# lzhLab/kmcEx

Hardware: AMD Instinct MI355X
Metric: k-mers/s encoded (insert) + k-mers/s queried, k=31 nh=7; % HBM-BW roofline (higher is better)
Workload: dtype u64; 1 GPU; synthetic 100000000 distinct canonical 31-mers per GPU, D1 counts, insert then query (110000000 queries: all inserted k-mers shuffled, half reverse-complemented, +10% absent); k=31, nh=7, nb=5, ci=1, cs=1023, kmers_per_gpu=100000000

## Files before the change

kmcex_amd/csrc/kernels.hip:

```cpp
#include "launchers.h"
#include <cstdlib>

__constant__ u32 c_seeds[128] = {
	46757, 46769, 46771, 46807, 46811, 46817, 46819, 46829, 46831, 46853, 46861, 46867, 46877, 46889, 46901, 46919,
	46933, 46957, 46993, 46997, 47017, 47041, 47051, 47057, 47059, 47087, 47093, 47111, 47119, 47123, 47129, 47137,
	47143, 47147, 47149, 47161, 47189, 47207, 47221, 47237, 47251, 47269, 47279, 47287, 47293, 47297, 47303, 47309,
	47317, 47339, 47351, 47353, 47363, 47381, 47387, 47389, 47407, 47417, 47419, 47431, 47441, 47459, 47491, 47497,
	47501, 47507, 47513, 47521, 47527, 47533, 47543, 47563, 47569, 47581, 47591, 47599, 47609, 47623, 47629, 47639,
	47653, 47657, 47659, 47681, 47699, 47701, 47711, 47713, 47717, 47737, 47741, 47743, 47777, 47779, 47791, 47797,
	47807, 47809, 47819, 47837, 47843, 47857, 47869, 47881, 47903, 47911, 47917, 47933, 47939, 47947, 47951, 47963,
	47969, 47977, 47981, 48017, 48023, 48029, 48049, 48073, 48079, 48091, 48109, 48119, 48121, 48131, 48157, 48163};

template <int W> __device__ __forceinline__ void load_kmer(const u64 *base, u64 i, u64 *v)
{
#pragma unroll
	for (int w = 0; w < W; w++) v[w] = base[i * W + w];
}
template <int W> __device__ __forceinline__ void store_kmer(u64 *base, u64 i, const u64 *v)
{
#pragma unroll
	for (int w = 0; w < W; w++) base[i * W + w] = v[w];
}

template <int W> __device__ __forceinline__ void bloom_insert_pm(const Premixed<W> &pm, const StrGeom g, u32 *bits, const ModU64 md, int nhash)
// ... 1198 lines not shown
		for (int r = 0; r < RPT; r++) {
			if (!mine[r] && !ghost[r]) continue;
			const u32 pub = mine[r] ? resv[r] : (ghost[r] & hold[r]);
			u32 later = mine[r] ? 0u : (ghost[r] & ~hold[r]);
#pragma unroll
			for (int j = 0; j < NHM; j++)
				if (j < md.nh && ((pub >> j) & 1u)) {
					const u64 q = FIN_Q(r, j);
					u32 *slot = ((second[r] >> j) & 1u) ? s_t2 + fin_slot2(q) : s_t1 + fin_slot1(q);
					const u32 cur = *slot, mark = FIN_MARK | fin_ident(q) | (((bin[r] >> j) & 1u) << 30);
					if (!(cur & FIN_MARK)) *slot = mark;
					else if ((cur & 0x3FFFFFu) == fin_ident(q)) *slot = cur | mark;
					else later |= 1u << j;
				}
			if (mine[r]) {
				if (!defer) {
#pragma unroll
					for (int j = 0; j < NHM; j++)
						if (j < md.nh && ((resv[r] >> j) & 1u)) {
							const u32 b = FIN_BIT(r, j);
							atomicOr(cells + cidx[r][j], CELL_TAG(b) | (((bin[r] >> j) & 1u) ? CELL_VAL(b) : 0u));
						}
				}
				bd.status[pp][row + x[r]] = SLOT_INSERTED;
				live[r] = false;
				won[r] = true;
				succ++;
			}
			ghost[r] = later;
			if (later) s_pending[par] = 1;
			__builtin_amdgcn_sched_barrier(0);
		}
		lds_barrier();
#pragma unroll
		for (int r = 0; r < RPT; r++) {
			if (!live[r]) continue;
			bool conflict = false;
#pragma unroll
			for (int j = 0; j < NHM; j++)
				if (j < md.nh && ((resv[r] >> j) & 1u)) {
					const u64 q = FIN_Q(r, j);
					const u32 m = ((second[r] >> j) & 1u) ? s_t2[fin_slot2(q)] : s_t1[fin_slot1(q)];
					if ((m & FIN_MARK) && (m & 0x3FFFFFu) == fin_ident(q)) {
						conflict |= ((m >> 30) & 1u) != ((bin[r] >> j) & 1u);
						um[r] &= ~(1u << j);
					}
				}
			if (conflict) { mark_failed(bd, pp, i, row, x[r]); live[r] = false; }
			else s_pending[par] = 1;
			__builtin_amdgcn_sched_barrier(0);
		}
		lds_barrier();
#pragma unroll
		for (int r = 0; r < RPT; r++)
#pragma unroll
			for (int j = 0; j < NHM; j++)
				if (j < md.nh && ((resv[r] >> j) & 1u)) {
					const u64 q = FIN_Q(r, j);
					s_t1[fin_slot1(q)] = 0;
					if ((second[r] >> j) & 1u) s_t2[fin_slot2(q)] = 0;
				}
		lds_barrier();
		if (!s_pending[par]) break;
	}
#undef FIN_BIT
#undef FIN_Q
#pragma unroll
	for (int r = 0; r < RPT; r++)
		if (won[r] && defer) bd.Urec[lv][(row + rec[r]) * (1 + W)] |= REC_WON;
	if (!defer) drain_vmem();
	if (succ) atomicAdd(s_succ, succ);
	return iters + 1;
}

template <int W, int NHM, int RPT>
__device__ __forceinline__ void finish_lds_ranges(const ModelDev &md, const BlockDev &bd, int pp, int i, int a, int lv, int n, bool snapshot,
                                                   u32 *s_t1, u32 *s_t2, u32 *s_list, int *s_count, int *s_pending, int *s_succ)
{
	constexpr int CAP = RPT * 1024;
	const u64 row = (u64)i * KMX_BUCKET;
	for (int q = threadIdx.x; q < KMX_FIN_T; q += 1024) { s_t1[q] = 0; s_t2[q] = 0; }
	u64 iters = 0;
	if (n <= CAP) {
		__syncthreads();
		iters = finish_lds<W, NHM, RPT>(md, bd, pp, i, a, lv, n, nullptr, snapshot, true, s_t1, s_t2, s_pending, s_succ);
	} else {
		const int n_list = bd.n[pp][i];
		int lo = 0, remaining = n;
		while (remaining > 0) {
			int hi = n_list;
			if (remaining > CAP) hi = lo + max(1, (int)((long long)(n_list - lo) * (CAP * 7 / 8) / remaining));
			int cnt;
			for (;;) {
				if (threadIdx.x == 0) *s_count = 0;
				__syncthreads();
				for (int u = threadIdx.x; u < n; u += 1024) {
					const int x = (int)((u32)bd.Urec[lv][(row + u) * (1 + W)] & (KMX_BUCKET - 1));
					if (x >= lo && x < hi) {
						const int slot = atomicAdd(s_count, 1);
						if (slot < CAP) s_list[slot] = (u32)u;
					}
				}
				__syncthreads();
				cnt = *s_count;
				__syncthreads();
				if (cnt <= CAP) break;
				hi = lo + max(1, (hi - lo) / 2);
			}
			iters += finish_lds<W, NHM, RPT>(md, bd, pp, i, a, lv, cnt, s_list, snapshot && lo == 0, false, s_t1, s_t2, s_pending, s_succ);
			__syncthreads();
			if (threadIdx.x == 0) s_pending[0] = 0;
			remaining -= cnt;
			lo = hi;
			if (lo >= n_list) break;
		}
	}
	__syncthreads();
	if (threadIdx.x == 0) {
		atomicAdd(bd.stats + ST_FIN_ITERS, iters);
		if (*s_succ) atomicAdd(bd.stats + ST_SLOW_SUCC, (u64)*s_succ);
	}
}

template <int W, int NHM>
__device__ __forceinline__ void finish_global(const ModelDev &md, const BlockDev &bd, int pp, int i, int a, int lv, int n, bool first, u64 epoch_b, u64 epoch0,
                                               int *s_pending, int *s_succ)
{
	const u64 row = (u64)i * KMX_BUCKET;
	u64 epoch = epoch0;
	u64 iters = 0;
	for (;; iters++) {
		if (threadIdx.x == 0) *s_pending = 0;
		__syncthreads();
		if (!first) {
			for (int u = threadIdx.x; u < n; u += 1024) {
				u32 x, bin;
				u64 v[W];
				rec_load<W>(bd.Urec[lv], row + u, x, bin, v);
				if (bd.status[pp][row + x] != SLOT_UNDECIDED) continue;
				Premixed<W> pm = premix_string<W>(left_align<W>(v, md.k), md.gfull);
				Touches<NHM> tc;
				gather_touches<W, NHM, true>(md, pm, a, tc);
				if (touches_conflict<NHM>(md, tc, bin)) { mark_failed(bd, pp, i, row, x); continue; }
				reserve_untagged<NHM>(md, bd, i, tc, resv_key(epoch, x));
				*s_pending = 1;
			}
			drain_vmem();
			__syncthreads();
			const int pending = *s_pending;
			__syncthreads();
			if (!pending) break;
		}
		int succ = 0;
		for (int u = threadIdx.x; u < n; u += 1024) {
			u32 x, bin;
			u64 v[W];
			const u32 um = rec_load<W>(bd.Urec[lv], row + u, x, bin, v);
			if (bd.status[pp][row + x] != SLOT_UNDECIDED) continue;
			Aligned<W> al = left_align<W>(v, md.k);
			Premixed<W> pm = premix_string<W>(al, md.gfull);
			if (first) {
				const u64 key = resv_key(epoch_b, x);
				const int sbase = a * md.nh;
				cell_t *cells = md.cells[a];
				u64 pos[NHM];
				bool mine = true;
#pragma unroll
				for (int j = 0; j < NHM; j++)
					if (j < md.nh && ((um >> j) & 1u)) {
						pos[j] = mod_u64(murmur_seeded<W>(pm, md.gfull, c_seeds[(sbase + j) & 127]), md.km_mod);
						mine &= cell_load_coherent(resv_slot(bd, i, pos[j])) == key;
					}
				if (mine) {
#pragma unroll
					for (int j = 0; j < NHM; j++)
						if (j < md.nh && ((um >> j) & 1u)) {
							const u32 b = bit_in_cell(pos[j]);
							atomicOr(cells + (pos[j] >> 4), CELL_TAG(b) | (value_at_position<NHM>(md, pos, um, bin, j) ? CELL_VAL(b) : 0u));
						}
					bd.status[pp][row + x] = SLOT_INSERTED;
					succ++;
				}
				continue;
			}
			Touches<NHM> tc;
			gather_touches<W, NHM, true>(md, pm, a, tc);
			if (owns_outcome<NHM, true>(md, bd, i, tc, bin, resv_key(epoch, x))) {
				commit_touches<W, NHM>(md, tc, bin, a);
				bd.status[pp][row + x] = SLOT_INSERTED;
				succ++;
			}
		}
		if (succ) atomicAdd(s_succ, succ);
		drain_vmem();
		__syncthreads();
		if (!first) epoch++;
		first = false;
	}
	if (threadIdx.x == 0) {
		atomicAdd(bd.stats + ST_FIN_ITERS, iters);
		if (*s_succ) atomicAdd(bd.stats + ST_SLOW_SUCC, (u64)*s_succ);
	}
}

template <int W, int NHM> __global__ __launch_bounds__(1024) void k_slow_finish(ModelDev md, BlockDev bd, int t, int pp, int s, u64 epoch_b, u64 epoch0, int force_global, KmbackJob job, BitScatter kmb)
{
	constexpr int RKPT = KMX_FIN_RIDER_KPT(NHM);
	constexpr int FIN_BYTES = (2 * KMX_FIN_T + KMX_FIN_RPT(NHM) * 1024) * 4 + 8 * 4, RIDER_BYTES = BS_LDS_BYTES(RKPT * (NHM - 2), 1024);
	__shared__ __align__(16) unsigned char pool[FIN_BYTES > RIDER_BYTES ? FIN_BYTES : RIDER_BYTES];
	if ((int)blockIdx.x >= md.nb) {
		const int r = (int)blockIdx.x - md.nb, gxk = KMX_BUCKET / (1024 * RKPT);
		kmback_emit_body<W, NHM, RKPT, 1024>(md, bd, job.kmers, job.surv, pp, job.n_in_block, kmb, job.i0 + r / gxk, r % gxk, gxk, pool);
		return;
	}
	u32 *s_t1 = (u32 *)pool, *s_t2 = s_t1 + KMX_FIN_T, *s_list = s_t2 + KMX_FIN_T;
	int *s_pending = (int *)(s_list + KMX_FIN_RPT(NHM) * 1024);
	int &s_succ = s_pending[3], &s_count = s_pending[4];
	const int i = blockIdx.x, lv = s & 1;
	const int n = bd.Un[UN_IDX(lv, i, md.nb)];
	if (n == 0) return;
	const int a = (i + t) % md.nb;
	constexpr int RPT = KMX_FIN_RPT(NHM);
	const bool lds_path = n <= KMX_FIN_RANGES * RPT * 1024 && !force_global && md.km_mod.d < KMX_FIN_MAX_POS;
	if (threadIdx.x == 0) {
		s_succ = 0;
		s_pending[0] = 0;
		atomicMax(bd.stats + ST_MAX_UFIN, (u64)n);
		if (s == 0) { atomicAdd(bd.stats + ST_CONTENDED, (u64)n); atomicMax(bd.stats + ST_MAX_U0, (u64)n); }
	}
	__syncthreads();
	const bool snap = s == 0 && snapshot_ok(bd, i);
	if (lds_path) finish_lds_ranges<W, NHM, RPT>(md, bd, pp, i, a, lv, n, snap, s_t1, s_t2, s_list, &s_count, s_pending, &s_succ);
	else finish_global<W, NHM>(md, bd, pp, i, a, lv, n, snap, epoch_b, epoch0, s_pending, &s_succ);
}

template <int W, int NHM> __global__ __launch_bounds__(256) void k_reorder(ModelDev md, BlockDev bd, int t, int pp, int lv)
{
	__shared__ int s_tmp[4];
	__shared__ int s_m, s_off;
	const int nb = md.nb;
	const int i = blockIdx.y, tile = blockIdx.x;
	const int n = bd.n[pp][i];
	const u64 row = (u64)i * KMX_BUCKET;
	if (tile >= (int)KMX_NTILES) {
		const int nrec = bd.Un[UN_IDX(lv, i, nb)];
		for (int u = (tile - (int)KMX_NTILES) * 256 + threadIdx.x; u < nrec; u += KMX_APPLY_WGS * 256) {
			const u64 *rec = bd.Urec[lv] + (row + u) * (1 + W);
			if (rec[0] & REC_WON) {
				const int a = (i + t) % nb;
				u32 x, bin;
				u64 v[W];
				rec_load<W>(bd.Urec[lv], row + u, x, bin, v);
				Aligned<W> al = left_align<W>(v, md.k);
				Premixed<W> pm = premix_string<W>(al, md.gfull);
				cell_t *cells = md.cells[a];
#pragma unroll
				for (int j = 0; j < NHM; j++)
					if (j < md.nh) {
						const u64 pos = mod_u64(murmur_seeded<W>(pm, md.gfull, c_seeds[(a * md.nh + j) & 127]), md.km_mod);
						const u32 b = bit_in_cell(pos);
						atomicOr(cells + (pos >> 4), CELL_TAG(b) | (((bin >> j) & 1u) ? CELL_VAL(b) : 0u));
					}
			}
		}
		return;
	}
	{
		int c = bd.tile_cnt[pp][i * KMX_NTILES + threadIdx.x];
		int tot;
		int ex = block_excl_scan_256(c, s_tmp, &tot);
		if ((int)threadIdx.x == tile) s_off = ex;
		if (threadIdx.x == 0) s_m = tot;
		__syncthreads();
	}
	const int m = s_m;
	int f[4], c = 0;
#pragma unroll
	for (int q = 0; q < 4; q++) {
		int x = tile * KMX_TILE + threadIdx.x * 4 + q;
		f[q] = (x < n && bd.status[pp][row + x] == SLOT_FAILED) ? 1 : 0;
		c += f[q];
	}
	int before = block_excl_scan_256(c, s_tmp, nullptr) + s_off;
	const u32 *oldl = bd.list[pp] + row;
	u32 *newl = bd.list[pp ^ 1] + row;
	u32 *mv = bd.mover[pp ^ 1] + row;
#pragma unroll
	for (int q = 0; q < 4; q++) {
		int x = tile * KMX_TILE + threadIdx.x * 4 + q;
		if (x < n) {
			if (x < m) newl[x] = f[q] ? oldl[x] : (LIST_HOLE | (u32)(x - before));
			else if (f[q]) mv[m - before - 1] = oldl[x];
		}
		before += f[q];
	}
	bd.tile_cnt[pp ^ 1][i * KMX_NTILES + tile] = 0;
	if (tile == 0 && threadIdx.x == 0) {
		bd.cl_ovf[i] = 0;
		if (n > m) atomicAdd(bd.stats + ST_SUCCESSES, (u64)(n - m));
		bd.n[pp ^ 1][i] = m;
	}
}

__global__ __launch_bounds__(1024) void k_bs_apply(BitScatter bs)
{
	__shared__ u32 s_tile[BS_TILE_WORDS];
	const u32 TW = 1u << (bs.tlog2 - 5);
	const u32 b = blockIdx.x;
	u32 cnt = (u32)bs.cnt[b];
	if (cnt == 0) return;
	if (cnt > bs.cap) cnt = bs.cap;
	const u64 wpb = 1ULL << (bs.wshift - 5), word0 = (u64)b * wpb;
	if (word0 >= bs.nwords) return;
	const u32 nw = (u32)((bs.nwords - word0) < wpb ? (bs.nwords - word0) : wpb);
	const u32 *tup = bs.tup + (u64)b * bs.cap;
	u32 *words = bs.words + word0;
	for (u32 t0 = 0; t0 < nw; t0 += TW) {
		const u32 tw = nw - t0 < TW ? nw - t0 : TW;
		for (u32 w = threadIdx.x; w < tw; w += 1024) s_tile[w] = 0;
		__syncthreads();
		for (u32 q = threadIdx.x; q < cnt; q += 1024) {
			const u32 o = tup[q], w = (o >> 5) - t0;
			if (w < tw) atomicOr(&s_tile[w], 1u << (o & 31));
		}
		__syncthreads();
		for (u32 w = threadIdx.x; w < tw; w += 1024) {
			const u32 x = s_tile[w];
			if (x) words[t0 + w] |= x;
		}
		__syncthreads();
	}
	if (threadIdx.x == 0) bs.cnt[b] = 0;
}

#define BS_SPLIT_K 8
__global__ __launch_bounds__(256) void k_bs_split(BitScatter bs)
{
	__shared__ int s_cnt[1 << BS_MAX_TILES_LOG2], s_off[1 << BS_MAX_TILES_LOG2], s_base[1 << BS_MAX_TILES_LOG2], s_tmp[4];
	__shared__ u32 s_stage[256 * BS_SPLIT_K];
	const u32 b = blockIdx.y, tl = bs.wshift - bs.tlog2, tmask = (1u << bs.tlog2) - 1;
	u32 cnt = (u32)bs.cnt[b];
	if (cnt > bs.cap) cnt = bs.cap;
	const u32 *tup = bs.tup + (u64)b * bs.cap;
	u32 *out = bs.tup2 + (((u64)b << tl) * bs.cap2);
	int *gcnt = bs.cnt2 + ((u64)b << tl);
	for (u32 base = blockIdx.x * (256 * BS_SPLIT_K); base < cnt; base += gridDim.x * (256 * BS_SPLIT_K)) {
		s_cnt[threadIdx.x] = 0;
		__syncthreads();
		u32 o[BS_SPLIT_K];
		int rank[BS_SPLIT_K];
#pragma unroll
		for (int j = 0; j < BS_SPLIT_K; j++) {
			const u32 q = base + j * 256 + threadIdx.x;
			o[j] = q < cnt ? tup[q] : ~0u;
		}
#pragma unroll
		for (int j = 0; j < BS_SPLIT_K; j++)
			if (o[j] != ~0u) rank[j] = atomicAdd(&s_cnt[o[j] >> bs.tlog2], 1);
		__syncthreads();
		int total;
		{
			const int c = s_cnt[threadIdx.x];
			const int ex = block_excl_scan_256(c, s_tmp, &total);
			s_off[threadIdx.x] = ex;
			s_base[threadIdx.x] = c ? atomicAdd(gcnt + threadIdx.x, c) : 0;
		}
		__syncthreads();
#pragma unroll
		for (int j = 0; j < BS_SPLIT_K; j++)
			if (o[j] != ~0u) s_stage[s_off[o[j] >> bs.tlog2] + rank[j]] = o[j];
		__syncthreads();
		for (int q = threadIdx.x; q < total; q += 256) {
			const u32 e = s_stage[q], t = e >> bs.tlog2;
			const u32 g = (u32)s_base[t] + (u32)(q - s_off[t]);
			if (g < bs.cap2) out[(u64)t * bs.cap2 + g] = e & tmask;
			else atomicOr(bs.words + (((u64)b << bs.wshift) >> 5) + (e >> 5), 1u << (e & 31));
		}
		__syncthreads();
	}
}
__global__ __launch_bounds__(1024) void k_bs_apply2(BitScatter bs)
{
	__shared__ u32 s_tile[BS_TILE_WORDS];
	const u32 b = blockIdx.y, t = blockIdx.x, tl = bs.wshift - bs.tlog2, TW = 1u << (bs.tlog2 - 5);
	int *gc = bs.cnt2 + (((u64)b << tl) + t);
	u32 cnt = (u32)*gc;
	if (t == 0 && threadIdx.x == 0) bs.cnt[b] = 0;
	if (cnt == 0) return;
	if (cnt > bs.cap2) cnt = bs.cap2;
	const u64 word0 = (((u64)b << bs.wshift) >> 5) + (u64)t * TW;
	if (word0 >= bs.nwords) { if (threadIdx.x == 0) *gc = 0; return; }
	const u32 tw = (u32)((bs.nwords - word0) < TW ? (bs.nwords - word0) : TW);
	const u32 *tup = bs.tup2 + (((u64)b << tl) + t) * bs.cap2;
	u32 *words = bs.words + word0;
	for (u32 w = threadIdx.x; w < tw; w += 1024) s_tile[w] = 0;
	__syncthreads();
	for (u32 q = threadIdx.x; q < cnt; q += 1024) {
		const u32 o = tup[q];
		if ((o >> 5) < tw) atomicOr(&s_tile[o >> 5], 1u << (o & 31));
	}
	__syncthreads();
	for (u32 w = threadIdx.x; w < tw; w += 1024) {
		const u32 x = s_tile[w];
		if (x) words[w] |= x;
	}
	if (threadIdx.x == 0) *gc = 0;
}

template <int W, int NHM, int KPT, int BT>
__device__ __forceinline__ void kmback_emit_body(const ModelDev &md, const BlockDev &bd, const u64 *kmers, const unsigned char *surv, int pp, int n_in_block,
                                                 const BitScatter &bs, int i, int bx, int gx, unsigned char *lds)
{
	constexpr int K = KPT * (NHM - 2);
	BS_LDS_AT(K, BT, lds);
	const bool whole = n_in_block >= 0;
	int n;
	if (whole) { n = n_in_block - i * (int)KMX_BUCKET; n = n < 0 ? 0 : (n > (int)KMX_BUCKET ? (int)KMX_BUCKET : n); }
	else n = bd.n[pp][i];
	const u64 row = (u64)i * KMX_BUCKET;
	for (int base = bx * BT * KPT; base < n; base += gx * BT * KPT) {
		u64 v[K];
		u32 valid = 0;
#pragma unroll
		for (int q = 0; q < KPT; q++) {
			const int x = base + q * BT + (int)threadIdx.x;
			if (x < n && (whole ? !surv[row + x] : bd.status[pp][row + x] != SLOT_FAILED)) {
				const u32 idx = whole ? (u32)x : bd.list[pp][row + x];
				u64 km[W];
				load_kmer<W>(kmers, row + idx, km);
				Premixed<W> pb = premix_string<W>(drop_first_base<W>(left_align<W>(km, md.k)), md.gback);
				if (md.kmb_direct) {
					bloom_insert_pm<W>(pb, md.gback, md.km_back, md.km_back_mod, md.nh - 2);
					continue;
				}
#pragma unroll
				for (int j = 0; j < NHM - 2; j++)
					if (j < md.nh - 2) {
						const u64 pos = mod_u64(murmur_seeded<W>(pb, md.gback, c_seeds[j]), md.km_back_mod);
						v[q * (NHM - 2) + j] = ((pos >> 5) << 5) | bit_in_word32(pos);
						valid |= 1u << (q * (NHM - 2) + j);
					}
			}
		}
		if (!md.kmb_direct) bs_block_emit<K, BT>(bs, v, valid, s_bs_cnt, s_bs_off, s_bs_base, s_bs_tmp, s_bs_stage);
	}
}
template <int W, int NHM, int KPT> __global__ __launch_bounds__(256) void k_kmback_emit(ModelDev md, BlockDev bd, const u64 *kmers, const unsigned char *surv, int i0, int istride, int pp, int n_in_block, BitScatter bs)
{
	__shared__ __align__(16) unsigned char lds[BS_LDS_BYTES(KPT * (NHM - 2), 256)];
	kmback_emit_body<W, NHM, KPT>(md, bd, kmers, surv, pp, n_in_block, bs, i0 + (int)blockIdx.y * istride, (int)blockIdx.x, (int)gridDim.x, lds);
}

template <int W> __global__ __launch_bounds__(256) void k_rest_append(BlockDev bd, int pp, int i0, int istride, u64 *rest_kmers, int *rest_counts, unsigned long long *rest_n, u64 *stale_kmers, int *stale_counts, u64 *feedback)
{
	__shared__ int s_cnt;
	__shared__ unsigned long long s_base;
	if (blockIdx.x == 0 && blockIdx.y == 0 && threadIdx.x == 0) {
		feedback[0] = bd.stats[ST_MAX_U0]; feedback[1] = bd.stats[ST_MAX_UFIN]; feedback[2] = bd.stats[ST_MAX_LATE_BIN];
		bd.stats[ST_MAX_U0] = 0; bd.stats[ST_MAX_UFIN] = 0; bd.stats[ST_MAX_LATE_BIN] = 0;
	}
	if (threadIdx.x == 0) s_cnt = 0;
	__syncthreads();
	const int i = i0 + (int)blockIdx.y * istride, x = blockIdx.x * 256 + threadIdx.x;
	const int n = bd.n[pp][i];
	if (x == 0 && n == 0) stale_counts[i] = 0;
	const bool act = x < n;
	const u64 mask = __ballot(act);
	const int lane = threadIdx.x & 63;
	int wbase = 0;
	if (lane == 0 && mask) wbase = atomicAdd(&s_cnt, (int)__popcll(mask));
	wbase = __shfl(wbase, 0, 64);
	__syncthreads();
	if (threadIdx.x == 0) s_base = s_cnt ? atomicAdd(rest_n, (unsigned long long)s_cnt) : 0ULL;
	__syncthreads();
	if (!act) return;
	const u64 p = s_base + (u64)wbase + (u64)__popcll(mask & ((1ULL << lane) - 1));
	const u64 row = (u64)i * KMX_BUCKET;
	const u32 idx = list_entry(bd, pp, row, x);
	u64 v[W];
	load_kmer<W>(bd.kmers, row + idx, v);
	const int c = (int)bd.counts[row + idx];
	store_kmer<W>(rest_kmers, p, v);
	rest_counts[p] = c;
	bd.surv[row + idx] = 1;
	if (x == 0) { store_kmer<W>(stale_kmers, (u64)i, v); stale_counts[i] = c; }
}

template <int W> __global__ __launch_bounds__(256) void k_ring_import(BlockDev bd, int nb, int pp, RingLists rl, u64 *stg_kmers, u32 *stg_counts)
{
	const int i = blockIdx.y, x = blockIdx.x * 256 + threadIdx.x;
	const RingList e = rl.e[i];
	const u64 row = (u64)i * KMX_BUCKET;
	int n = 0;
	if (e.active) {
		const u64 *src_k = e.n_host >= 0 ? e.src_kmers : e.src_msg + KMX_MSG_HDR;
		const u32 *src_c = e.n_host >= 0 ? e.src_counts : (const u32 *)(e.src_msg + KMX_MSG_HDR + (u64)KMX_BUCKET * W);
		n = e.n_host >= 0 ? e.n_host : (int)e.src_msg[0];
		n = n < 0 ? 0 : (n > (int)KMX_BUCKET ? (int)KMX_BUCKET : n);
		if (x < n) {
			u64 v[W];
			load_kmer<W>(src_k, (u64)x, v);
			store_kmer<W>(stg_kmers, row + x, v);
			stg_counts[row + x] = src_c[x];
		}
		bd.list[pp][row + x] = (u32)x;
		bd.surv[row + x] = 0;
	}
	if (x < (int)KMX_NTILES) { bd.tile_cnt[0][i * KMX_NTILES + x] = 0; bd.tile_cnt[1][i * KMX_NTILES + x] = 0; }
	if (x == 0) {
		bd.n[pp][i] = n;
		for (int s = 0; s < KMX_NSLOW; s++) bd.Un[UN_IDX(s, i, nb)] = 0;
	}
}

template <int W> __global__ __launch_bounds__(256) void k_ring_export(BlockDev bd, int pp, RingLists rl, u64 *feedback)
{
	const int i = blockIdx.y, x = blockIdx.x * 256 + threadIdx.x;
	if (blockIdx.x == 0 && blockIdx.y == 0 && threadIdx.x == 0) {
		const u64 late = bd.stats[ST_MAX_LATE_BIN];
		if (late && late > feedback[2]) feedback[2] = late;
	}
	const RingList e = rl.e[i];
	if (!e.active || !e.dst_msg) return;
	const int n = bd.n[pp][i];
	const u64 row = (u64)i * KMX_BUCKET;
	if (x == 0) e.dst_msg[0] = (u64)n;
	if (x >= n) return;
	const u32 idx = list_entry(bd, pp, row, x);
	u64 v[W];
	load_kmer<W>(bd.kmers, row + idx, v);
	store_kmer<W>(e.dst_msg + KMX_MSG_HDR, (u64)x, v);
	((u32 *)(e.dst_msg + KMX_MSG_HDR + (u64)KMX_BUCKET * W))[x] = bd.counts[row + idx];
}

__global__ __launch_bounds__(256) void k_or_words(u32 *dst, const u32 *src, u64 n)
{
	for (u64 i = (u64)blockIdx.x * 256 + threadIdx.x; i < n; i += (u64)gridDim.x * 256) {
		const u32 s = src[i];
		if (s) dst[i] |= s;
	}
}

template <int W> __device__ __forceinline__ u64 shr128_lo(const u64 *v, int s)
{
	if (W == 1) return s >= 64 ? 0 : v[0] >> s;
	if (s >= 64) return s >= 128 ? 0 : v[0] >> (s - 64);
	return s ? (v[0] << (64 - s)) | (v[1] >> s) : v[1];
}

template <int W> __device__ __forceinline__ int rest_check_reference(const ModelDev &md, u32 pre, const u64 *key)
{
	const int g = md.rest_h2i[pre];
	if (g < 0) return 0;
	int low = md.rest_pre[g], high = md.rest_pre[g + 1], mid = 0;
	bool found = false;
	while (low <= high) {
		mid = (low + high) / 2;
		if ((u64)mid >= md.rest_entries) break;
		int c = 0;
#pragma unroll
		for (int w = 0; w < W; w++) {
			u64 r = md.rest_suf[(u64)mid * W + w];
			if (c == 0) c = key[w] < r ? -1 : (key[w] > r ? 1 : 0);
		}
		if (c < 0) high = mid - 1;
		else if (c > 0) low = mid + 1;
		else { found = true; break; }
	}
	return found ? md.rest_cnt[mid] : 0;
}

template <int W> __device__ __forceinline__ int rest_check(const ModelDev &md, const u64 *v)
{
	if (!md.rest_entries) return 0;
	const int sbits = 2 * (md.k - md.rest_pre_len);
	const u32 pre = (u32)shr128_lo<W>(v, sbits);
	u64 key[W];
	if (W == 1) key[0] = v[0] & ((1ULL << sbits) - 1);
	else {
		if (sbits >= 64) { key[0] = sbits >= 128 ? v[0] : v[0] & ((1ULL << (sbits - 64)) - 1); key[W - 1] = v[W - 1]; }
		else { key[0] = 0; key[W - 1] = v[W - 1] & ((1ULL << sbits) - 1); }
	}
	const u32 b = (u32)shr128_lo<W>(v, 2 * md.k - md.rest_fbits);
	u32 lo = md.rest_fine[b], hi = md.rest_fine[b + 1];
	while (hi - lo > 4) {
		const u32 mid = (lo + hi) >> 1;
		bool less = false, eq = true;
#pragma unroll
		for (int w = 0; w < W; w++) {
			const u64 r = md.rest_suf[(u64)mid * W + w];
			if (eq && r != key[w]) { less = r < key[w]; eq = false; }
		}
		if (eq) return md.rest_cnt[mid];
		if (less) lo = mid + 1; else hi = mid;
	}
	for (u32 e = lo; e < hi; e++) {
		bool eq = true;
#pragma unroll
		for (int w = 0; w < W; w++) eq &= md.rest_suf[(u64)e * W + w] == key[w];
		if (eq) return md.rest_cnt[e];
	}
	bool q_eq = true;
#pragma unroll
	for (int w = 0; w < W; w++) q_eq &= md.rest_q[(u64)pre * W + w] == key[w];
	return q_eq ? rest_check_reference<W>(md, pre, key) : 0;
}

template <int PW> __device__ __forceinline__ int check_all_bf(const ModelDev &md, const StrGeom gf, const StrGeom gb, const Premixed<PW> &pf, const Premixed<PW> &pb)
{
	for (int j = 0; j < md.bf_num; j++) {
		int i = md.ci == 1 ? j : (j == 0 ? 1 : (j == 1 ? 0 : 2));
		bool a = bloom_check_pm<PW>(pf, gf, md.bf[i], md.bf_mod[i], md.nh - 1);
		bool b = a && bloom_check_pm<PW>(pb, gb, md.bf_back[i], md.bf_back_mod[i], md.nh - 2);
		if (a && b) return i + md.ci;
	}
	return 0;
}

template <int PW> __device__ __forceinline__ int decode_array(const ModelDev &md, const StrGeom gf, const Premixed<PW> &pf, int a)
{
	if (!md.km_mod.d) return -1;
	const cell_t *cells = md.cells[a];
	int v = 0;
	bool ok = true;
	for (int j = 0; j < md.nh && ok; j++) {
		u64 pos = mod_u64(murmur_seeded<PW>(pf, gf, c_seeds[(a * md.nh + j) & 127]), md.km_mod);
		const cell_t cell = cells[pos >> 4];
		u32 b = bit_in_cell(pos);
		ok = (cell >> (16 + b)) & 1u;
		v |= (int)((cell >> b) & 1u) << j;
	}
	return ok ? v : -1;
}
// ... 950 lines not shown
```

Measured before the change: 1.505 billion k-mers/s.

## Vectorize bit-scatter apply with uint4 loads, prefetched words, fewer barriers

```diff
diff --git a/kmcex_amd/csrc/kernels.hip b/kmcex_amd/csrc/kernels.hip
--- a/kmcex_amd/csrc/kernels.hip
+++ b/kmcex_amd/csrc/kernels.hip
@@ -1524,9 +1524,16 @@
 	}
 }
 
+#define BS_SWEEP_LOADS 4
+#define BS_TILE_VECS (BS_TILE_WORDS / 4 / 1024)
+__device__ __forceinline__ void bs_tile_or(u32 *s_tile, u32 o, u32 t0, u32 tw)
+{
+	const u32 w = (o >> 5) - t0;
+	if (w < tw) atomicOr(&s_tile[w], 1u << (o & 31));
+}
 __global__ __launch_bounds__(1024) void k_bs_apply(BitScatter bs)
 {
-	__shared__ u32 s_tile[BS_TILE_WORDS];
+	__shared__ __align__(16) u32 s_tile[BS_TILE_WORDS];
 	const u32 TW = 1u << (bs.tlog2 - 5);
 	const u32 b = blockIdx.x;
 	u32 cnt = (u32)bs.cnt[b];
@@ -1537,20 +1544,68 @@
 	const u32 nw = (u32)((bs.nwords - word0) < wpb ? (bs.nwords - word0) : wpb);
 	const u32 *tup = bs.tup + (u64)b * bs.cap;
 	u32 *words = bs.words + word0;
+	u32 head = (u32)((16 - ((uintptr_t)tup & 15)) & 15) >> 2;
+	if (head > cnt) head = cnt;
+	const u32 nvec = (cnt - head) >> 2, nedge = cnt - 4 * nvec;
+	const uint4 *tup4 = (const uint4 *)(tup + head);
+	const bool wide = ((uintptr_t)words & 15) == 0;
+	uint4 *s_tile4 = (uint4 *)s_tile;
+	for (u32 i = threadIdx.x, n4 = ((nw < TW ? nw : TW) + 3) >> 2; i < n4; i += 1024) s_tile4[i] = make_uint4(0, 0, 0, 0);
+	__syncthreads();
 	for (u32 t0 = 0; t0 < nw; t0 += TW) {
-		const u32 tw = nw - t0 < TW ? nw - t0 : TW;
-		for (u32 w = threadIdx.x; w < tw; w += 1024) s_tile[w] = 0;
-		__syncthreads();
-		for (u32 q = threadIdx.x; q < cnt; q += 1024) {
-			const u32 o = tup[q], w = (o >> 5) - t0;
-			if (w < tw) atomicOr(&s_tile[w], 1u << (o & 31));
-		}
-		__syncthreads();
-		for (u32 w = threadIdx.x; w < tw; w += 1024) {
-			const u32 x = s_tile[w];
-			if (x) words[t0 + w] |= x;
-		}
-		__syncthreads();
+		const u32 tw = nw - t0 < TW ? nw - t0 : TW, tw4 = wide ? tw >> 2 : 0;
+		const bool more = t0 + TW < nw;
+		uint4 *words4 = (uint4 *)(words + t0);
+		for (u32 base = 0; base < nvec; base += 1024 * BS_SWEEP_LOADS) {
+			uint4 v[BS_SWEEP_LOADS];
+#pragma unroll
+			for (int j = 0; j < BS_SWEEP_LOADS; j++) {
+				const u32 i = base + j * 1024 + threadIdx.x;
+				v[j] = tup4[i < nvec ? i : nvec - 1];
+			}
+#pragma unroll
+			for (int j = 0; j < BS_SWEEP_LOADS; j++)
+				if (base + j * 1024 + threadIdx.x < nvec) {
+					bs_tile_or(s_tile, v[j].x, t0, tw);
+					bs_tile_or(s_tile, v[j].y, t0, tw);
+					bs_tile_or(s_tile, v[j].z, t0, tw);
+					bs_tile_or(s_tile, v[j].w, t0, tw);
+				}
+		}
+		if (threadIdx.x < nedge) bs_tile_or(s_tile, tup[threadIdx.x < head ? threadIdx.x : 4 * nvec + threadIdx.x], t0, tw);
+		uint4 old[BS_TILE_VECS], x[BS_TILE_VECS];
+#pragma unroll
+		for (int j = 0; j < BS_TILE_VECS; j++) {
+			const u32 i = j * 1024 + threadIdx.x;
+			old[j] = make_uint4(0, 0, 0, 0);
+			if (i < tw4) old[j] = words4[i];
+		}
+		__syncthreads();
+#pragma unroll
+		for (int j = 0; j < BS_TILE_VECS; j++) {
+			const u32 i = j * 1024 + threadIdx.x;
+			x[j] = make_uint4(0, 0, 0, 0);
+			if (i < tw4) x[j] = s_tile4[i];
+		}
+#pragma unroll
+		for (int j = 0; j < BS_TILE_VECS; j++)
+			if (x[j].x | x[j].y | x[j].z | x[j].w)
+				words4[j * 1024 + threadIdx.x] = make_uint4(old[j].x | x[j].x, old[j].y | x[j].y, old[j].z | x[j].z, old[j].w | x[j].w);
+		if (more) {
+#pragma unroll
+			for (int j = 0; j < BS_TILE_VECS; j++) {
+				const u32 i = j * 1024 + threadIdx.x;
+				if (i < tw4) s_tile4[i] = make_uint4(0, 0, 0, 0);
+			}
+		}
+		for (u32 w = 4 * tw4 + threadIdx.x; w < tw; w += 1024) {
+			const u32 y = s_tile[w];
+			if (y) {
+				words[t0 + w] |= y;
+				if (more) s_tile[w] = 0;
+			}
+		}
+		if (more) __syncthreads();
 	}
 	if (threadIdx.x == 0) bs.cnt[b] = 0;
 }
```

Measured after the change: 1.533 billion k-mers/s, median of 6. +1.8%, better.
